# TheRealShamsaba/KnightVision

Hardware: AMD Instinct MI355X
Metric: MCTS simulations/sec + self-play games/hour (higher is better)
Workload: dtype fp32

## Files before the change

### include/kv.h

```cpp
#ifndef KV_H
#define KV_H

#include <stddef.h>
#include <stdint.h>

#ifdef __cplusplus
extern "C" {
#endif

#define KV_OK 0
#define KV_EINVAL -1
#define KV_ENOMEM -2
#define KV_EHIP -3
#define KV_EOVERFLOW -4

const char* kv_last_error(void);
int kv_version(void);

typedef struct kv_net kv_net;

size_t kv_net_packed_size(void);
int kv_net_create(int device, kv_net** out);
int kv_net_load(kv_net* net, const float* packed, size_t n_floats);
int kv_net_forward(kv_net* net, const float* planes_dev, int B, float* policy_dev, float* value_dev, void* stream);
// ... 174 lines not shown
size_t kv_sizeof_search_result(void);

int kv_search_advance(kv_engine* e, int n, const int32_t* edge , int8_t* states_out );
int kv_search_continue(kv_engine* e, int n, const kv_search_params* p, kv_search_result* out ,
                       int32_t* kept );
int kv_search_tree_size(kv_engine* e, int i, int32_t* nodes, int32_t* edges);


int kv_dev_valid_moves(int device, const int8_t* states, int n, uint16_t* moves_out, int cap, int* n_moves,
                       int8_t* states_after, uint8_t* in_check);
int kv_dev_attacks(int device, const int8_t* states, int n, uint64_t* attacked);
int kv_dev_make_move(int device, int8_t* states, const int* index, int n);
int kv_dev_dirichlet(int device, const uint64_t* seeds, int n, double alpha, int k, int draws, double* out,
                     int64_t* attempts, double* tail);
int kv_dev_eval_cache(int device, int entries, const int8_t* boards, const uint16_t* moves, const int* counts,
                      const uint32_t* logits, const uint32_t* values, int n_rows, const int* step_len, int n_steps,
                      int32_t* hit, uint32_t* out_logits, uint32_t* out_values, int64_t* counters);
int kv_host_libm(int op, const double* x, const double* y, int n, double* out);
int kv_dev_py_random(int device, const uint64_t* seeds, int n, int count, double* out);
int kv_dev_wino88i(int device, const double* V, int rows, const double* U, int K, int digits, int seg, double* M,
                   int8_t* v_digits, int* v_exp);
int kv_dev_wino88i32_out(int device, const float* M, int rows, const float* scale, const float* shift,
                         const float* resid, int fused, float* Y, int8_t* v_digits, int* v_exp);
int kv_dev_tower_front(int device, const int8_t* boards, int nb, int rows, const float* wT, const float* scale,
                       const float* shift, int fused, int8_t* v_digits, int* v_exp);
int kv_dev_tower_back(int device, const float* M, int rows, const float* scale, const float* shift,
                      const float* resid, const float* heads, int fused, float* pfeat, float* value);
int kv_dev_wino88r_out(int device, const double* M, int rows, const float* scale, const float* shift,
                       const float* resid, int fused, float* Y, int8_t* v_digits, int* v_exp);
int kv_dev_net_pair(kv_net* a, kv_net* b, int cu_share, int follow);
int kv_dev_i8gemm_bench(int device, int rows, int K, int variant, int iters, float* avg_us, float* M_out);
int kv_dev_gemm_clock(int device, int rows, int digits, double seconds, double* out);
int kv_dev_out_phases(int device, int rows, int resid, int r3, unsigned long long* stamps, float* us);

#define KV_PGN_OUTCOME_NONE (-128)
typedef struct kv_pgn_record {
    char fen[100];
    char san[12];
    int32_t outcome;
    int32_t game;
} kv_pgn_record;
int kv_pgn_extract(const char* text, size_t len, kv_pgn_record* out, size_t cap, size_t* n_out, size_t* consumed,
                   int64_t* n_games);
int kv_fen_codes(const char* fens, size_t stride, int n, int8_t* codes);
int kv_san_move_index(const char* fens, size_t fen_stride, const char* sans, size_t san_stride, int n,
                      int32_t* out);
int kv_chess_perft(const char* fen, int depth, uint64_t* nodes);
int kv_chess_san(const char* fen, const char* san_in, char* san_out, size_t san_cap, char* fen_after, size_t fen_cap);
int kv_chess_fen(const char* fen_in, char* fen_out, size_t cap);

int kv_tr_conv3x3_f16(const void* x_dev, int n, int ci, const void* w_dev, const float* bias_dev, int co,
                      void* y_dev, void* stream);
int kv_tr_conv3x3_add_f16(const void* x_dev, int n, int ci, const void* w_dev, const float* bias_dev, int co,
                          const void* add_dev, void* y_dev, void* stream);
int kv_tr_conv_weights_f16(const float* w_dev, int co, int ci_real, int ci, void* wf_dev, void* wt_dev, void* stream);
size_t kv_tr_wgrad_workspace(int n, int ci, int co, int* splits);
int kv_tr_conv3x3_wgrad_f16(const void* dy_dev, const void* x_dev, int n, int ci, int ci_real, int co, float* dw_dev,
                            void* ws_dev, size_t ws_bytes, void* stream);
size_t kv_tr_bn_workspace(int rows, int C);
int kv_tr_bn_stats_f16(const void* x_dev, int rows, int C, float eps, float* mean_dev, float* var_dev,
                       float* invstd_dev, void* ws_dev, size_t ws_bytes, void* stream);
int kv_tr_bn_apply_f16(const void* x_dev, int rows, int C, const float* mean_dev, const float* invstd_dev,
                       const float* gamma_dev, const float* beta_dev, const void* res_dev, int relu, void* y_dev,
                       void* stream);
int kv_tr_bn_backward_f16(const void* x_dev, const void* dy_dev, const void* y_dev, int rows, int C, int relu,
                          const float* mean_dev, const float* invstd_dev, const float* gamma_dev, float* dgamma_dev,
// ... 23 lines not shown
```

### knightvision_amd/_lib.py

```python
from __future__ import annotations

import ctypes as C
import os

HERE = os.path.dirname(os.path.abspath(__file__))
LIB_PATH = os.environ.get("KV_LIB_PATH") or os.path.join(HERE, "libkv.so")

_lib = None


class KVError(RuntimeError):
    pass


class Config(C.Structure):
    _fields_ = [("device", C.c_int), ("slots", C.c_int), ("n_games", C.c_int64), ("game_id_base", C.c_int64),
                ("game_id_stride", C.c_int64), ("seed", C.c_uint64), ("seed_mode", C.c_int),
                ("max_moves", C.c_int), ("batch", C.c_int), ("eps", C.c_double), ("alpha", C.c_double),
                ("sims", C.c_int), ("c_puct", C.c_float), ("eval_mode", C.c_int), ("record_cap", C.c_int64),
                ("recycle", C.c_int), ("precision", C.c_int), ("algo", C.c_int), ("tree_edge_cap", C.c_int),
                ("keep_root_visits", C.c_int), ("eval_cache", C.c_int), ("leaves", C.c_int), ("arena", C.c_int), ("sample_plies", C.c_int),
                ("sim_groups", C.c_int), ("reuse_tree", C.c_int)]


# ... 96 lines not shown
        "kv_run": ([vp, i64, i64], i),
        "kv_set_max_moves": ([vp, i], i),
        "kv_records": ([vp, P(Record), sz, P(sz)], i),
        "kv_games": ([vp, P(Game), sz, P(sz)], i),
        "kv_stats_get": ([vp, P(Stats)], i),
        "kv_sizeof_config": ([], sz),
        "kv_sizeof_stats": ([], sz),
        "kv_root_visits": ([vp, P(C.c_int32), sz, P(sz)], i),
        "kv_root_visits_device": ([vp, vp, sz, P(sz), vp], i),
        "kv_root_moves": ([vp, P(C.c_uint16), sz, P(sz)], i),
        "kv_root_moves_device": ([vp, vp, sz, P(sz), vp], i),
        "kv_records_device": ([vp, vp, sz, P(sz), vp], i),
        "kv_sync": ([vp], i),
        "kv_reset_records": ([vp], i),
        "kv_destroy": ([vp], None),
        "kv_search": ([vp, P(C.c_int8), i, P(SearchParams), P(SearchResult)], i),
        "kv_sizeof_search_result": ([], sz),
        "kv_search_advance": ([vp, i, P(C.c_int32), P(C.c_int8)], i),
        "kv_search_continue": ([vp, i, P(SearchParams), P(SearchResult), P(C.c_int32)], i),
        "kv_search_tree_size": ([vp, i, P(C.c_int32), P(C.c_int32)], i),
        "kv_dev_valid_moves": ([i, P(C.c_int8), i, P(C.c_uint16), i, P(i), P(C.c_int8), P(C.c_uint8)], i),
        "kv_dev_make_move": ([i, P(C.c_int8), P(i), i], i),
        "kv_dev_attacks": ([i, P(C.c_int8), i, P(C.c_uint64)], i),
        "kv_dev_dirichlet": ([i, P(C.c_uint64), i, C.c_double, i, i, P(C.c_double), P(i64), P(C.c_double)], i),
        "kv_dev_py_random": ([i, P(C.c_uint64), i, i, P(C.c_double)], i),
        "kv_dev_eval_cache": ([i, i, P(C.c_int8), P(C.c_uint16), P(i), P(C.c_uint32), P(C.c_uint32), i, P(i), i,
                               P(C.c_int32), P(C.c_uint32), P(C.c_uint32), P(i64)], i),
        "kv_host_libm": ([i, P(C.c_double), P(C.c_double), i, P(C.c_double)], i),
        "kv_dev_wino88i": ([i, P(C.c_double), i, P(C.c_double), i, i, i, P(C.c_double), P(C.c_int8), P(i)], i),
        "kv_dev_i8gemm_bench": ([i, i, i, i, i, P(C.c_float), P(C.c_float)], i),
        "kv_dev_gemm_clock": ([i, i, i, C.c_double, P(C.c_double)], i),
        "kv_dev_net_pair": ([vp, vp, i, i], i),
        "kv_dev_out_phases": ([i, i, i, i, P(C.c_uint64), P(C.c_float)], i),
        "kv_dev_wino88i32_out": ([i, P(C.c_float), i, P(C.c_float), P(C.c_float), P(C.c_float), i, P(C.c_float),
                                  P(C.c_int8), P(i)], i),
        "kv_dev_tower_front": ([i, P(C.c_int8), i, i, P(C.c_float), P(C.c_float), P(C.c_float), i, P(C.c_int8),
                                P(i)], i),
        "kv_dev_tower_back": ([i, P(C.c_float), i, P(C.c_float), P(C.c_float), P(C.c_float), P(C.c_float), i,
                               P(C.c_float), P(C.c_float)], i),
        "kv_dev_wino88r_out": ([i, P(C.c_double), i, P(C.c_float), P(C.c_float), P(C.c_float), i, P(C.c_float),
                                P(C.c_int8), P(i)], i),
        "kv_pgn_extract": ([C.c_char_p, sz, P(PgnRecord), sz, P(sz), P(sz), P(i64)], i),
        "kv_fen_codes": ([C.c_char_p, sz, i, P(C.c_int8)], i),
        "kv_san_move_index": ([C.c_char_p, sz, C.c_char_p, sz, i, P(C.c_int32)], i),
        "kv_chess_perft": ([C.c_char_p, i, P(C.c_uint64)], i),
        "kv_chess_san": ([C.c_char_p, C.c_char_p, C.c_char_p, sz, C.c_char_p, sz], i),
        "kv_chess_fen": ([C.c_char_p, C.c_char_p, sz], i),
        "kv_tr_conv3x3_f16": ([vp, i, i, vp, vp, i, vp, vp], i),
        "kv_tr_conv3x3_add_f16": ([vp, i, i, vp, vp, i, vp, vp, vp], i),
        "kv_tr_conv_weights_f16": ([vp, i, i, i, vp, vp, vp], i),
        "kv_tr_wgrad_workspace": ([i, i, i, P(i)], sz),
        "kv_tr_conv3x3_wgrad_f16": ([vp, vp, i, i, i, i, vp, vp, sz, vp], i),
        "kv_tr_bn_workspace": ([i, i], sz),
        "kv_tr_bn_stats_f16": ([vp, i, i, C.c_float, vp, vp, vp, vp, sz, vp], i),
        "kv_tr_bn_apply_f16": ([vp, i, i, vp, vp, vp, vp, vp, i, vp, vp], i),
        "kv_tr_bn_backward_f16": ([vp, vp, vp, i, i, i, vp, vp, vp, vp, vp, vp, vp, vp, vp, sz, vp], i),
        "kv_tr_channel_sum_f16": ([vp, i, i, vp, vp, sz, vp], i),
        "kv_tr_planes_to_nhwc": ([vp, i, i, vp, vp], i),
        "kv_tr_head1x1_f16": ([vp, i, vp, vp, vp, vp], i),
        "kv_tr_head1x1_workspace": ([i], sz),
        "kv_tr_head1x1_backward_f16": ([vp, vp, i, vp, vp, vp, vp, vp, sz, vp], i),
        "kv_tr_policy_loss_f16": ([vp, vp, vp, vp, vp, i, vp, vp, vp, vp], i),
        "kv_tr_policy_loss_backward_f16": ([vp, vp, vp, vp, vp, i, vp, vp, vp, vp, vp, vp], i),
    }
    for name, (args, res) in sig.items():
        if not hasattr(L, name):
            continue
        f = getattr(L, name)
        f.argtypes = args
        f.restype = res
    return L


EXPORTED = ["kv_last_error", "kv_version", "kv_net_packed_size", "kv_net_create", "kv_net_load", "kv_net_forward",
            "kv_net_forward_boards", "kv_net_forward_boards_legal", "kv_net_set_timing", "kv_net_last_timing", "kv_net_destroy", "kv_net_set_precision", "kv_net_set_algo",
            "kv_net_calibration", "kv_engine_calibration",
            "kv_create", "kv_sim_groups_for",
            "kv_load_weights", "kv_load_weights_b", "kv_engine_calibration_b", "kv_run", "kv_set_max_moves", "kv_records", "kv_games", "kv_stats_get", "kv_sizeof_config", "kv_sizeof_stats", "kv_root_visits", "kv_root_visits_device", "kv_root_moves", "kv_root_moves_device", "kv_records_device", "kv_sync", "kv_reset_records", "kv_destroy",
            "kv_search", "kv_sizeof_search_result", "kv_search_advance", "kv_search_continue", "kv_search_tree_size",
            "kv_dev_valid_moves", "kv_dev_make_move", "kv_dev_attacks", "kv_dev_dirichlet", "kv_dev_py_random", "kv_host_libm", "kv_dev_eval_cache",
            "kv_dev_wino88i", "kv_dev_wino88i32_out", "kv_dev_wino88r_out", "kv_dev_tower_front", "kv_dev_tower_back", "kv_dev_i8gemm_bench",
            "kv_dev_gemm_clock", "kv_dev_out_phases", "kv_dev_net_pair",
            "kv_pgn_extract", "kv_fen_codes", "kv_san_move_index", "kv_chess_perft", "kv_chess_san", "kv_chess_fen",
            "kv_tr_conv3x3_f16", "kv_tr_conv3x3_add_f16", "kv_tr_conv_weights_f16", "kv_tr_wgrad_workspace", "kv_tr_conv3x3_wgrad_f16",
            "kv_tr_bn_workspace", "kv_tr_bn_stats_f16", "kv_tr_bn_apply_f16", "kv_tr_bn_backward_f16",
            "kv_tr_channel_sum_f16", "kv_tr_planes_to_nhwc", "kv_tr_head1x1_f16", "kv_tr_head1x1_workspace",
            "kv_tr_head1x1_backward_f16", "kv_tr_policy_loss_f16", "kv_tr_policy_loss_backward_f16"]


def lib():
    global _lib
    if _lib is None:
        import torch
        if not os.path.exists(LIB_PATH):
            raise KVError(f"{LIB_PATH} is missing: run `python -c 'import __graft_entry__ as g; g.build()'` "
                          "(the HIP library is required; there is no CPU fallback)")
        L = _declare(C.CDLL(LIB_PATH))
        if hasattr(L, "kv_sizeof_search_result"):
            assert L.kv_sizeof_search_result() == C.sizeof(SearchResult), "kv_search_result: ctypes mirror differs"
        if hasattr(L, "kv_sizeof_config"):
            assert L.kv_sizeof_config() == C.sizeof(Config), "kv_config: ctypes mirror differs"
            assert L.kv_sizeof_stats() == C.sizeof(Stats), "kv_stats: ctypes mirror differs"
        _lib = L
    return _lib


def check(rc: int, what: str = ""):
    if rc != 0:
        msg = lib().kv_last_error().decode(errors="replace")
        raise KVError(f"{what} failed ({rc}): {msg}")
```

### knightvision_amd/csrc/kv_nn.hip

```cpp
#include <hip/hip_runtime.h>
#include <math.h>
#include <stdarg.h>
#include <stdlib.h>
#include <string.h>

#include <algorithm>
#include <chrono>
#include <mutex>
#include <set>
#include <utility>
#include <vector>

#include "kv_common.h"
#include "kv_wino.h"
#include "kv_wino88.h"
#include "kv_wino88d.h"
#include "kv_wino88i.h"
#include "kv_ref64.h"

namespace kv {

static thread_local char g_err[512];

void set_error(const char* fmt, ...) {
// ... 2547 lines not shown
    kv::DevEvent e0, e1;
    KV_HIP(e0.create());
    KV_HIP(e1.create());
    for (int it = 0; it < 4; ++it) {
        if (it == 3) KV_HIP(hipEventRecord(e0.e, 0));
        if (resid && r3)
            hipLaunchKernelGGL((kv::wino88i32_out_kernel<true, true, 512, true, true>), dim3(1, rows), dim3(1024), 0, 0,
                               dm.p, rows, dsc.p, dsh.p, dy.p, dy.p, v8.p, ev.p, 0, 0);
        else if (resid)
            hipLaunchKernelGGL((kv::wino88i32_out_kernel<true, true, 512, false, true>), dim3(1, rows), dim3(1024), 0,
                               0, dm.p, rows, dsc.p, dsh.p, dy.p, dy.p, v8.p, ev.p, 0, 0);
        else if (r3)
            hipLaunchKernelGGL((kv::wino88i32_out_kernel<false, false, 512, true, true>), dim3(1, rows), dim3(1024), 0,
                               0, dm.p, rows, dsc.p, dsh.p, nullptr, nullptr, v8.p, ev.p, 0, 0);
        else
            hipLaunchKernelGGL((kv::wino88i32_out_kernel<false, false, 512, false, true>), dim3(1, rows), dim3(1024), 0,
                               0, dm.p, rows, dsc.p, dsh.p, nullptr, nullptr, v8.p, ev.p, 0, 0);
        KV_HIP(hipGetLastError());
    }
    KV_HIP(hipEventRecord(e1.e, 0));
    KV_HIP(hipEventSynchronize(e1.e));
    float ms = 0.f;
    KV_HIP(hipEventElapsedTime(&ms, e0.e, e1.e));
    *us = 1000.f * ms;
    const int nb = rows < kv::kOutStampBoards ? rows : kv::kOutStampBoards;
    std::vector<unsigned long long> h((size_t)kv::kOutStampBoards * 16);
    KV_HIP(hipMemcpyFromSymbol(h.data(), HIP_SYMBOL(kv::kOutStamps), h.size() * sizeof(unsigned long long)));
    for (int b = 0; b < nb; ++b)
        for (int w = 0; w < 2; ++w)
            for (int k = 0; k < 6; ++k) stamps[((size_t)b * 2 + w) * 6 + k] = h[((size_t)b * 2 + w) * 8 + k];
    return KV_OK;
}

int kv_dev_net_pair(kv_net* a, kv_net* b, int cu_share, int follow) {
    KV_REQUIRE(a && b && a != b && cu_share >= 1 && cu_share <= 2, KV_EINVAL, "kv_dev_net_pair: bad argument");
    KV_REQUIRE(a->device == b->device, KV_EINVAL, "kv_dev_net_pair: the nets are on different devices");
    KV_HIP(hipSetDevice(a->device));
    a->cu_share = b->cu_share = cu_share;
    a->leader = nullptr;
    b->leader = follow ? a : nullptr;
    if (follow)
        for (int l = 1; l < 12; ++l)
            if (!a->gemm_done[l]) KV_HIP(hipEventCreateWithFlags(&a->gemm_done[l], hipEventDisableTiming));
    return KV_OK;
}

int kv_net_set_timing(kv_net* net, int enable) {
    KV_REQUIRE(net, KV_EINVAL, "kv_net_set_timing: NULL");
    net->timing = enable != 0;
    return KV_OK;
}

int kv_net_last_timing(kv_net* net, float* conv_ms, int* n_conv) {
    KV_REQUIRE(net && net->timing, KV_EINVAL, "kv_net_last_timing: timing not enabled");
    KV_HIP(hipEventSynchronize(net->ev[2]));
    float ms = 0.f;
    KV_HIP(hipEventElapsedTime(&ms, net->ev[1], net->ev[2]));
    if (conv_ms) *conv_ms = ms;
    if (n_conv) *n_conv = 10;
    return KV_OK;
}

void kv_net_destroy(kv_net* net) {
    if (!net || net->view) return;
    (void)hipSetDevice(net->device);
    (void)hipFree(net->w);
// ... 105 lines not shown
```

### knightvision_amd/csrc/kv_wino88.h

```cpp
#pragma once
#include <hip/hip_runtime.h>

#include "kv_common.h"
#include "kv_wino.h"

namespace kv {

constexpr int W88_XI = 100;

__device__ inline void w88_bt(const float* d, float* o) {
#pragma clang fp contract(off)
    o[0] = __builtin_fmaf(1.0f, d[8], __builtin_fmaf(-6.362500190734863f, d[6], __builtin_fmaf(10.802399635314941f, d[4], __builtin_fmaf(-5.5696001052856445f, d[2], 0.6399999856948853f * d[0]))));
    o[1] = __builtin_fmaf(1.0f, d[8], __builtin_fmaf(0.4000000059604645f, d[7], __builtin_fmaf(-6.202499866485596f, d[6], __builtin_fmaf(-2.4809999465942383f, d[5], __builtin_fmaf(9.8100004196167f, d[4], __builtin_fmaf(3.9240000247955322f, d[3], __builtin_fmaf(-4.0f, d[2], -1.600000023841858f * d[1])))))));
    o[2] = __builtin_fmaf(1.0f, d[8], __builtin_fmaf(-0.4000000059604645f, d[7], __builtin_fmaf(-6.202499866485596f, d[6], __builtin_fmaf(2.4809999465942383f, d[5], __builtin_fmaf(9.8100004196167f, d[4], __builtin_fmaf(-3.9240000247955322f, d[3], __builtin_fmaf(-4.0f, d[2], 1.600000023841858f * d[1])))))));
    o[3] = __builtin_fmaf(1.0f, d[8], __builtin_fmaf(0.800000011920929f, d[7], __builtin_fmaf(-5.722499847412109f, d[6], __builtin_fmaf(-4.578000068664551f, d[5], __builtin_fmaf(7.139999866485596f, d[4], __builtin_fmaf(5.711999893188477f, d[3], __builtin_fmaf(-1.0f, d[2], -0.800000011920929f * d[1])))))));
    o[4] = __builtin_fmaf(1.0f, d[8], __builtin_fmaf(-0.800000011920929f, d[7], __builtin_fmaf(-5.722499847412109f, d[6], __builtin_fmaf(4.578000068664551f, d[5], __builtin_fmaf(7.139999866485596f, d[4], __builtin_fmaf(-5.711999893188477f, d[3], __builtin_fmaf(-1.0f, d[2], 0.800000011920929f * d[1])))))));
    o[5] = __builtin_fmaf(1.0f, d[8], __builtin_fmaf(1.25f, d[7], __builtin_fmaf(-4.800000190734863f, d[6], __builtin_fmaf(-6.0f, d[5], __builtin_fmaf(3.3024001121520996f, d[4], __builtin_fmaf(4.127999782562256f, d[3], __builtin_fmaf(-0.40959998965263367f, d[2], -0.5120000243186951f * d[1])))))));
    o[6] = __builtin_fmaf(1.0f, d[8], __builtin_fmaf(-1.25f, d[7], __builtin_fmaf(-4.800000190734863f, d[6], __builtin_fmaf(6.0f, d[5], __builtin_fmaf(3.3024001121520996f, d[4], __builtin_fmaf(-4.127999782562256f, d[3], __builtin_fmaf(-0.40959998965263367f, d[2], 0.5120000243186951f * d[1])))))));
    o[7] = __builtin_fmaf(1.0f, d[8], __builtin_fmaf(2.0f, d[7], __builtin_fmaf(-2.362499952316284f, d[6], __builtin_fmaf(-4.724999904632568f, d[5], __builtin_fmaf(1.3523999452590942f, d[4], __builtin_fmaf(2.7047998905181885f, d[3], __builtin_fmaf(-0.1599999964237213f, d[2], -0.3199999928474426f * d[1])))))));
    o[8] = __builtin_fmaf(1.0f, d[8], __builtin_fmaf(-2.0f, d[7], __builtin_fmaf(-2.362499952316284f, d[6], __builtin_fmaf(4.724999904632568f, d[5], __builtin_fmaf(1.3523999452590942f, d[4], __builtin_fmaf(-2.7047998905181885f, d[3], __builtin_fmaf(-0.1599999964237213f, d[2], 0.3199999928474426f * d[1])))))));
    o[9] = __builtin_fmaf(1.0f, d[9], __builtin_fmaf(-6.362500190734863f, d[7], __builtin_fmaf(10.802399635314941f, d[5], __builtin_fmaf(-5.5696001052856445f, d[3], 0.6399999856948853f * d[1]))));
}

__device__ inline void w88_at(const float* d, float* o) {
// ... 154 lines not shown
#pragma clang fp contract(off)
    constexpr int C = 512;
    const size_t xs = (size_t)rows * C;
    const size_t base = (size_t)b * C + c;
    float tmp[8][10];
#pragma unroll
    for (int j = 0; j < 10; ++j) {
        float col[10], o[8];
#pragma unroll
        for (int i = 0; i < 10; ++i) col[i] = __builtin_nontemporal_load(&M[(size_t)(i * 10 + j) * xs + base]);
        w88_at(col, o);
#pragma unroll
        for (int i = 0; i < 8; ++i) tmp[i][j] = o[i];
    }
    float res[64];
#pragma unroll
    for (int p = 0; p < 64; ++p) res[p] = RESID ? resid[((size_t)b * 64 + p) * C + c] : 0.f;
#pragma unroll
    for (int i = 0; i < 8; ++i) {
        float o[8];
        w88_at(tmp[i], o);
#pragma unroll
        for (int j = 0; j < 8; ++j) {
            const int p = i * 8 + j;
            float v = o[j] * sc + sh;
            if (RESID) v += res[p];
            v = v > 0.f ? v : 0.f;
            if (WRITE_Y) Y[((size_t)b * 64 + p) * C + c] = v;
            x[p] = v;
        }
    }
}

#ifndef KV_OUT_M_NT
#define KV_OUT_M_NT 1
#endif
template <bool RESID, bool WRITE_Y, bool STAGED = false, int ABL = 0, bool YNT = false>
__device__ inline void wino88_out_plane_half(const float* __restrict__ M, int rows, int b, int c, int h, float sc,
                                             float sh, const float* resid, float* Y, float (&x2)[4][8]) {
#pragma clang fp contract(off)
    constexpr int C = 512;
    const unsigned xs = (unsigned)rows * C;
    const unsigned base = (unsigned)b * C + c;
    float t[8][5];
    unsigned rbase = (unsigned)b * 64 * C + c;
    if constexpr (STAGED) {
        unsigned mb = base;
#pragma unroll
        for (int jj = 0; jj < 5; ++jj) {
            const int j = 5 * h + jj;
            float col[10];
#pragma unroll
            for (int i = 0; i < 10; ++i) col[i] = __builtin_nontemporal_load(&M[(unsigned)(i * 10 + j) * xs + mb]);
            float o[8];
            w88_at(col, o);
#pragma unroll
            for (int i = 0; i < 8; ++i) t[i][jj] = o[i];
            asm volatile("" : "+v"(mb) : "v"(o[0]), "v"(o[7]));
        }
        asm volatile("" : "+v"(rbase) : "v"(t[0][4]), "v"(t[7][4]));
    } else if constexpr (ABL == 1) {
        const int wv = (int)(threadIdx.x >> 6), ln = (int)(threadIdx.x & 63);
        f32x4 q[13];
#pragma unroll
        for (int k = 0; k < 13; ++k) {
            const int g = wv * 13 + k, xi = (g >> 1) < 99 ? (g >> 1) : 99;
            q[k] = __builtin_nontemporal_load(
                (const f32x4*)&M[(unsigned)xi * xs + (unsigned)b * C + (unsigned)((g & 1) * 256 + 4 * ln)]);
        }
#pragma unroll
        for (int jj = 0; jj < 5; ++jj) {
            float col[10], o[8];
#pragma unroll
            for (int i = 0; i < 10; ++i) col[i] = q[(jj * 10 + i) >> 2][(jj * 10 + i) & 3];
            w88_at(col, o);
#pragma unroll
            for (int i = 0; i < 8; ++i) t[i][jj] = o[i];
        }
    } else {
#pragma unroll
        for (int jj = 0; jj < 5; ++jj) {
            const int j = 5 * h + jj;
            float col[10], o[8];
#pragma unroll
            for (int i = 0; i < 10; ++i)
                col[i] = KV_OUT_M_NT ? __builtin_nontemporal_load(&M[(unsigned)(i * 10 + j) * xs + base])
                                     : M[(unsigned)(i * 10 + j) * xs + base];
            w88_at(col, o);
#pragma unroll
            for (int i = 0; i < 8; ++i) t[i][jj] = o[i];
        }
    }
#pragma unroll
    for (int ii = 0; ii < 4; ++ii) {
        float row[10];
#pragma unroll
        for (int jj = 0; jj < 5; ++jj) {
            float lo = t[ii][jj], hi = t[4 + ii][jj];
            half_swap(lo, hi);
            row[jj] = lo;
            row[5 + jj] = hi;
        }
        float o[8];
        w88_at(row, o);
        const int i = 4 * h + ii;
        float res[8];
#pragma unroll
        for (int j = 0; j < 8; ++j)
            res[j] = RESID ? (YNT ? __builtin_nontemporal_load(&resid[(unsigned)(i * 8 + j) * C + rbase])
                                          : resid[(unsigned)(i * 8 + j) * C + rbase])
                           : 0.f;
#pragma unroll
        for (int j = 0; j < 8; ++j) {
            float v = o[j] * sc + sh;
            if (RESID) v += res[j];
            v = v > 0.f ? v : 0.f;
            if (WRITE_Y) {
                if (YNT)
                    __builtin_nontemporal_store(v, &Y[((unsigned)b * 64 + i * 8 + j) * C + c]);
                else
                    Y[((unsigned)b * 64 + i * 8 + j) * C + c] = v;
            }
            x2[ii][j] = v;
        }
        if (STAGED) asm volatile("" : "+v"(rbase) : "v"(x2[ii][0]), "v"(x2[ii][7]));
    }
}

template <bool RESID, bool WRITE_Y, bool NEXT_V>
__global__ __launch_bounds__(256) void wino88_out_kernel(const float* __restrict__ M, int rows,
                                                         const float* __restrict__ scale,
                                                         const float* __restrict__ shift, const float* resid, float* Y,
                                                         float* __restrict__ Vn) {
    constexpr int C = 512;
    const int c = blockIdx.x * 256 + threadIdx.x, b = blockIdx.y;
    float x[64];
    wino88_out_plane<RESID, WRITE_Y>(M, rows, b, c, scale[c], shift[c], resid, Y, x);
    if (NEXT_V) wino88_input_plane(x, Vn, (size_t)b * C + c, (size_t)rows * C);
}

}
```

### knightvision_amd/csrc/kv_wino88i.h

```cpp
#pragma once
#include <hip/hip_runtime.h>

#include "kv_common.h"
#include "kv_wino88.h"
#include "kv_wino88d.h"

namespace kv {

constexpr int kI8Digits = 5;
constexpr int kI8DigitsF32 = 4;

typedef int i8x16_t __attribute__((ext_vector_type(4)));
typedef int i32x16_t __attribute__((ext_vector_type(16)));

__device__ inline int i8_row_exponent(unsigned m) {
    if (!m) return 0;
    return (int)(m >> 20) - 1022 + ((m & 0xFE000u) == 0xFE000u ? 1 : 0);
}

__device__ inline int i8_row_exponent_f32(unsigned m) {
    if (!m) return 0;
    return (int)(m >> 23) - 126 + ((m & 0x7F0000u) == 0x7F0000u ? 1 : 0);
}

// ... 1610 lines not shown
        const int xi = threadIdx.x, a = xi / 10, bb = xi % 10, hh = a / 5, aa = a % 5;
        unsigned m = 0;
#pragma unroll
        for (int ww = 0; ww < NW; ++ww) m = red[ww][hh][aa][bb] > m ? red[ww][hh][aa][bb] : m;
        const int e = i8f32_row_exponent<R3>(m);
        exs[xi] = e;
        ex[(size_t)xi * rows + b] = e;
    }
    __syncthreads();
    const int q = lane & 3;
    const unsigned off0 = ((unsigned)(c >> 5) * rows + b) * kI8LineBytes<R3> + q * 32 + (c & 28),
                   xstride = NK * rows * kI8LineBytes<R3>;
    unsigned* const dst = (unsigned*)V8;
#pragma unroll
    for (int aa = 0; aa < 5; ++aa) {
        float o[10];
        wino88_input_row_of_cols(xc, aa, o);
        const int a = 5 * h + aa;
#pragma unroll
        for (int bb = 0; bb < 10; ++bb) {
            const int xi = a * 10 + bb;
            const unsigned P = i8f32_digits<R3>(o[bb], exs[xi]);
            {
                const unsigned T4 = i8_quad_transpose(P, lane);
                if constexpr (!R3)
                    __builtin_nontemporal_store(T4, &dst[(off0 + (unsigned)xi * xstride) >> 2]);
                else if (q < 3)
                    dst[(off0 + (unsigned)xi * xstride) >> 2] = T4;
            }
        }
    }
}

constexpr int kOutStampBoards = 4096;
__device__ unsigned long long kOutStamps[kOutStampBoards][2][8];

template <bool RESID, bool WRITE_Y, int CW, bool R3 = false, bool STAMP = false, int ABL = 0, bool YNT = false>
__global__ __launch_bounds__(2 * CW) void wino88i32_out_kernel(const float* __restrict__ M, int rows,
                                                               const float* __restrict__ scale,
                                                               const float* __restrict__ shift, const float* resid,
                                                               float* Y, int8_t* __restrict__ V8,
                                                               int* __restrict__ ex, int stag, int first) {
#pragma clang fp contract(off)
    static_assert(CW == 512 || CW == 256, "a row or a 256-channel segment per workgroup");
    constexpr int NK = 512 / 32, NW = CW / 32, NSEG = 512 / CW;
    __shared__ __attribute__((aligned(16))) unsigned red[NW][2][5][16];
    __shared__ int exs[100];
    const int lane = threadIdx.x & 63, w = threadIdx.x >> 6, h = lane >> 5;
    const int seg = blockIdx.x, c = seg * CW + w * 32 + (lane & 31), b = out_board<R3>((int)blockIdx.y);
    out_stagger(b, stag, first);
    unsigned long long st[6] = {};
    const bool stamper = STAMP && (w == 0 || w == NW - 1) && lane == 0 && b < kOutStampBoards;
    if constexpr (STAMP) st[0] = __builtin_amdgcn_s_memtime();
    float vk[5][10];
    {
        float t2[10][4];
        {
            float x2[4][8];
            wino88_out_plane_half<RESID, WRITE_Y, false, ABL, YNT>(M, rows, b, c, h, scale[c], shift[c], resid, Y, x2);
            wino88_input_cols(x2, h, t2);
        }
#pragma unroll
        for (int aa = 0; aa < 5; ++aa) wino88_input_row(t2, h, aa, vk[aa]);
    }
    if constexpr (STAMP) {
#pragma unroll
        for (int aa = 0; aa < 5; ++aa)
#pragma unroll
            for (int bb = 0; bb < 10; ++bb) asm volatile("" ::"v"(vk[aa][bb]));
        st[1] = __builtin_amdgcn_s_memtime();
    }
#pragma unroll
    for (int aa = 0; aa < 5; ++aa) {
        const float (&o)[10] = vk[aa];
        unsigned m[10];
#pragma unroll
        for (int bb = 0; bb < 10; ++bb) m[bb] = i8_half_max_dpp(__float_as_uint(o[bb]) & 0x7fffffffu);
        if ((lane & 31) == 16) {
            uint4* rr = (uint4*)&red[w][h][aa][0];
            rr[0] = make_uint4(m[0], m[1], m[2], m[3]);
            rr[1] = make_uint4(m[4], m[5], m[6], m[7]);
            *(uint2*)&red[w][h][aa][8] = make_uint2(m[8], m[9]);
        }
    }
    __syncthreads();
    if constexpr (STAMP) st[2] = __builtin_amdgcn_s_memtime();
    if (threadIdx.x < 100) {
        const int xi = threadIdx.x, a = xi / 10, bb = xi % 10, hh = a / 5, aa = a % 5;
        unsigned m = 0;
#pragma unroll
        for (int ww = 0; ww < NW; ++ww) m = red[ww][hh][aa][bb] > m ? red[ww][hh][aa][bb] : m;
        const int e = i8f32_row_exponent<R3>(m);
        exs[xi] = e;
        ex[((size_t)xi * NSEG + seg) * rows + b] = e;
    }
    __syncthreads();
    if constexpr (STAMP) st[3] = __builtin_amdgcn_s_memtime();
    const int q = lane & 3;
    const unsigned off0 = ((unsigned)(c >> 5) * rows + b) * kI8LineBytes<R3> + q * 32 + (c & 28),
                   xstride = NK * rows * kI8LineBytes<R3>;
    unsigned* const dst = (unsigned*)V8;
#pragma unroll
    for (int aa = 0; aa < 5; ++aa) {
        const int a = 5 * h + aa;
#pragma unroll
        for (int bb = 0; bb < 10; ++bb) {
            const int xi = a * 10 + bb;
            const unsigned P = i8f32_digits<R3>(vk[aa][bb], exs[xi]);
            {
                const unsigned T4 = i8_quad_transpose(P, lane);
                if constexpr (!R3)
                    __builtin_nontemporal_store(T4, &dst[(off0 + (unsigned)xi * xstride) >> 2]);
                else if (q < 3)
                    dst[(off0 + (unsigned)xi * xstride) >> 2] = T4;
            }
        }
    }
    if constexpr (STAMP) {
        st[4] = __builtin_amdgcn_s_memtime();
        asm volatile("s_waitcnt vmcnt(0)" ::: "memory");
        st[5] = __builtin_amdgcn_s_memtime();
        if (stamper) {
            unsigned long long* o = kOutStamps[b][w == 0 ? 0 : 1];
#pragma unroll
            for (int k = 0; k < 6; ++k) o[k] = st[k];
        }
    }
}

constexpr int kStemR3Lds = 9 * 13 * 256 * 4;
__global__ __launch_bounds__(512) void stem_r3_kernel(const int8_t* __restrict__ boards, int nb, int rows,
                                                      const float* __restrict__ wT, const float* __restrict__ scale,
                                                      const float* __restrict__ shift, int8_t* __restrict__ V8,
                                                      int* __restrict__ ex) {
#pragma clang fp contract(off)
    constexpr int NK = 256 / 32, NW = 8;
    extern __shared__ __attribute__((aligned(16))) float stem_wl[];
    __shared__ int codes[100];
    __shared__ __attribute__((aligned(16))) unsigned red[NW][2][5][16];
    __shared__ int exs[100];
    const int lane = threadIdx.x & 63, w = threadIdx.x >> 6, h = lane >> 5;
    const int c = w * 32 + (lane & 31);
    for (int i = threadIdx.x; i < 9 * 13 * 256; i += 512) {
        const int r = i >> 8, code = r / 9, t = r % 9;
        stem_wl[i] = code ? wT[(size_t)(t * 12 + code - 1) * 256 + (i & 255)] : 0.f;
    }
    const float sc = scale[c], sh = shift[c];
    const int q = lane & 3;
    unsigned* const dst = (unsigned*)V8;
    const unsigned xstride = NK * (unsigned)rows * 96u;
    for (int id = blockIdx.x; id < rows; id += gridDim.x) {
        const int b = out_board<true>(id);
        __syncthreads();
        if (threadIdx.x < 100) {
            const int i = threadIdx.x, r = i / 10 - 1, f = i % 10 - 1;
            const bool in = b < nb && r >= 0 && r < 8 && f >= 0 && f < 8;
            codes[i] = in ? boards[(size_t)b * 64 + r * 8 + f] * (9 * 256) : 0;
        }
        __syncthreads();
        float vk[5][10];
        {
            float t2[10][4];
            {
                float x2[4][8];
#pragma unroll
                for (int ii = 0; ii < 4; ++ii)
#pragma unroll
                    for (int px = 0; px < 8; ++px) {
                        const int py = 4 * h + ii;
                        float acc = 0.f;
#pragma unroll
                        for (int t = 0; t < 9; ++t)
                            acc += stem_wl[codes[(py + t / 3) * 10 + px + t % 3] + t * 256 + c];
                        const float v = __builtin_fmaf(acc, sc, sh);
                        x2[ii][px] = v > 0.f ? v : 0.f;
                    }
                wino88_input_cols(x2, h, t2);
            }
#pragma unroll
            for (int aa = 0; aa < 5; ++aa) wino88_input_row(t2, h, aa, vk[aa]);
        }
#pragma unroll
        for (int aa = 0; aa < 5; ++aa) {
            unsigned m[10];
#pragma unroll
            for (int bb = 0; bb < 10; ++bb) m[bb] = i8_half_max_dpp(__float_as_uint(vk[aa][bb]) & 0x7fffffffu);
            if ((lane & 31) == 16) {
                uint4* rr = (uint4*)&red[w][h][aa][0];
                rr[0] = make_uint4(m[0], m[1], m[2], m[3]);
                rr[1] = make_uint4(m[4], m[5], m[6], m[7]);
                *(uint2*)&red[w][h][aa][8] = make_uint2(m[8], m[9]);
            }
        }
        __syncthreads();
        if (threadIdx.x < 100) {
            const int xi = threadIdx.x, a = xi / 10, bb = xi % 10, hh = a / 5, aa = a % 5;
            unsigned m = 0;
#pragma unroll
            for (int ww = 0; ww < NW; ++ww) m = red[ww][hh][aa][bb] > m ? red[ww][hh][aa][bb] : m;
            const int e = i8_row_exponent_f32r(m);
            exs[xi] = e;
            ex[(size_t)xi * rows + b] = e;
        }
        __syncthreads();
        const unsigned off0 = ((unsigned)(c >> 5) * rows + b) * 96u + q * 32 + (c & 28);
#pragma unroll
        for (int aa = 0; aa < 5; ++aa) {
            const int a = 5 * h + aa;
#pragma unroll
            for (int bb = 0; bb < 10; ++bb) {
                const int xi = a * 10 + bb;
                const unsigned P = i8_digits_r3((double)vk[aa][bb], exs[xi]);
                const unsigned T4 = i8_quad_transpose(P, lane);
                if (q < 3) dst[(off0 + (unsigned)xi * xstride) >> 2] = T4;
            }
        }
    }
}

template <bool RESID, bool WRITE_Y, bool R3 = false>
__global__ __launch_bounds__(1024) void wino88i32_outp_kernel(const float* __restrict__ M, int rows,
                                                              const float* __restrict__ scale,
                                                              const float* __restrict__ shift, const float* resid,
                                                              float* Y, int8_t* __restrict__ V8,
                                                              int* __restrict__ ex) {
#pragma clang fp contract(off)
    constexpr int NK = 512 / 32, NW = 16, NSLOT = 3, SLOT = 20 * 2048;
    extern __shared__ __attribute__((aligned(16))) char lds_outp[];
    unsigned(*red)[2][5][16] = (unsigned(*)[2][5][16])(lds_outp + NSLOT * SLOT);
    int* exs = (int*)(lds_outp + NSLOT * SLOT + NW * 2 * 5 * 16 * 4);
    const int lane = threadIdx.x & 63, w = threadIdx.x >> 6, h = lane >> 5;
    const int wu = __builtin_amdgcn_readfirstlane(w);
    const int c = w * 32 + (lane & 31);
    const int G = (int)gridDim.x;
    const int nbw = ((int)rows - (int)blockIdx.x + G - 1) / G;
    const int nsteps = 5 * nbw;
    const int npieces = wu < 8 ? 3 : 2;
    const float sc = scale[c], sh = shift[c];
    const unsigned xs = (unsigned)rows * 512;
    auto issue = [&](int t) {
        if (t >= nsteps) return;
        const int b = (int)blockIdx.x + (t / 5) * G, jj = t % 5;
        char* dst = lds_outp + (t % NSLOT) * SLOT;
#pragma unroll
        for (int k = 0; k < 3; ++k) {
            const int q = wu + 16 * k;
            if (q < 40) {
                const int r = q >> 1, hh = r / 10, i = r - 10 * hh;
                const float* src = M + (unsigned)(i * 10 + 5 * hh + jj) * xs + (unsigned)b * 512 + (q & 1) * 256 +
// ... 244 lines not shown
```

Before: 336,700.

## Rework R3 output epilogue: permlane max reduction, f32 digit cut, scalar-base addressing

The per-row max reduction before quantisation now uses permlane16_swap plus a DPP tree, so every lane ends up holding two maxima, replacing fifty separate half-wave DPP reductions. Digit quantisation is done in f32 with precomputed shifts instead of a double-precision conversion, and the quad transpose uses precomputed perm selectors. Global loads and stores use a scalar base plus a per-lane offset, aiming to cut VGPR address arithmetic. A standalone benchmark entry point with ablation variants is also added; the f32 cut could round differently from the double path.

```diff
diff --git a/include/kv.h b/include/kv.h
--- a/include/kv.h
+++ b/include/kv.h
@@ -230,6 +230,7 @@
 int kv_dev_i8gemm_bench(int device, int rows, int K, int variant, int iters, float* avg_us, float* M_out);
 int kv_dev_gemm_clock(int device, int rows, int digits, double seconds, double* out);
 int kv_dev_out_phases(int device, int rows, int resid, int r3, unsigned long long* stamps, float* us);
+int kv_dev_out_bench(int device, int rows, int resid, int abl, int iters, float* us);
 
 #define KV_PGN_OUTCOME_NONE (-128)
 typedef struct kv_pgn_record {
diff --git a/knightvision_amd/_lib.py b/knightvision_amd/_lib.py
--- a/knightvision_amd/_lib.py
+++ b/knightvision_amd/_lib.py
@@ -152,6 +152,7 @@
         "kv_dev_gemm_clock": ([i, i, i, C.c_double, P(C.c_double)], i),
         "kv_dev_net_pair": ([vp, vp, i, i], i),
         "kv_dev_out_phases": ([i, i, i, i, P(C.c_uint64), P(C.c_float)], i),
+        "kv_dev_out_bench": ([i, i, i, i, i, P(C.c_float)], i),
         "kv_dev_wino88i32_out": ([i, P(C.c_float), i, P(C.c_float), P(C.c_float), P(C.c_float), i, P(C.c_float),
                                   P(C.c_int8), P(i)], i),
         "kv_dev_tower_front": ([i, P(C.c_int8), i, i, P(C.c_float), P(C.c_float), P(C.c_float), i, P(C.c_int8),
@@ -200,7 +201,7 @@
             "kv_search", "kv_sizeof_search_result", "kv_search_advance", "kv_search_continue", "kv_search_tree_size",
             "kv_dev_valid_moves", "kv_dev_make_move", "kv_dev_attacks", "kv_dev_dirichlet", "kv_dev_py_random", "kv_host_libm", "kv_dev_eval_cache",
             "kv_dev_wino88i", "kv_dev_wino88i32_out", "kv_dev_wino88r_out", "kv_dev_tower_front", "kv_dev_tower_back", "kv_dev_i8gemm_bench",
-            "kv_dev_gemm_clock", "kv_dev_out_phases", "kv_dev_net_pair",
+            "kv_dev_gemm_clock", "kv_dev_out_phases", "kv_dev_out_bench", "kv_dev_net_pair",
             "kv_pgn_extract", "kv_fen_codes", "kv_san_move_index", "kv_chess_perft", "kv_chess_san", "kv_chess_fen",
             "kv_tr_conv3x3_f16", "kv_tr_conv3x3_add_f16", "kv_tr_conv_weights_f16", "kv_tr_wgrad_workspace", "kv_tr_conv3x3_wgrad_f16",
             "kv_tr_bn_workspace", "kv_tr_bn_stats_f16", "kv_tr_bn_apply_f16", "kv_tr_bn_backward_f16",
diff --git a/knightvision_amd/csrc/kv_nn.hip b/knightvision_amd/csrc/kv_nn.hip
--- a/knightvision_amd/csrc/kv_nn.hip
+++ b/knightvision_amd/csrc/kv_nn.hip
@@ -2603,6 +2603,61 @@
     return KV_OK;
 }
 
+}
+
+template <bool RESID, int ABL>
+static void dev_out_bench_launch(const float* M, int rows, const float* sc, const float* sh, float* y, int8_t* v8,
+                                 int* ev, int cus) {
+    hipLaunchKernelGGL((kv::wino88i32_out_kernel<RESID, RESID, 512, true, false, ABL, RESID>), dim3(1, rows),
+                       dim3(1024), 0, 0, M, rows, sc, sh, RESID ? y : nullptr, RESID ? y : nullptr, v8, ev, 0, cus);
+}
+
+extern "C" {
+
+int kv_dev_out_bench(int device, int rows, int resid, int abl, int iters, float* us) {
+    KV_REQUIRE(rows > 0 && rows % 128 == 0 && rows <= kMaxBoards && us && iters > 0 && iters <= 1000 &&
+                   (abl == 0 || abl == 4 || abl == 8),
+               KV_EINVAL, "kv_dev_out_bench: bad arguments (rows %d, abl %d, iters %d)", rows, abl, iters);
+    KV_HIP(hipSetDevice(device));
+    const size_t nm = (size_t)kv::W88_XI * rows * 512, ny = (size_t)rows * 64 * 512;
+    kv::DevBuf<float> dm, dsc, dsh, dy;
+    kv::DevBuf<int8_t> v8;
+    kv::DevBuf<int> ev;
+    KV_HIP(dm.alloc(nm));
+    KV_HIP(dsc.alloc(512));
+    KV_HIP(dsh.alloc(512));
+    KV_HIP(dy.alloc(ny));
+    KV_HIP(v8.alloc(nm * 4));
+    KV_HIP(ev.alloc((size_t)kv::W88_XI * rows));
+    hipLaunchKernelGGL(out_phase_fill_kernel, dim3((unsigned)((nm + 255) / 256)), dim3(256), 0, 0, dm.p, nm, dsc.p,
+                       dsh.p);
+    KV_HIP(hipMemset(dy.p, 0, ny * sizeof(float)));
+    KV_HIP(hipGetLastError());
+    const int cus = device_cus();
+    std::vector<kv::DevEvent> e((size_t)iters + 1);
+    for (auto& x : e) KV_HIP(x.create());
+    for (int it = -3; it < iters; ++it) {
+        if (it == 0) KV_HIP(hipEventRecord(e[0].e, 0));
+        if (resid)
+            abl == 4   ? dev_out_bench_launch<true, 4>(dm.p, rows, dsc.p, dsh.p, dy.p, v8.p, ev.p, cus)
+            : abl == 8 ? dev_out_bench_launch<true, 8>(dm.p, rows, dsc.p, dsh.p, dy.p, v8.p, ev.p, cus)
+                       : dev_out_bench_launch<true, 0>(dm.p, rows, dsc.p, dsh.p, dy.p, v8.p, ev.p, cus);
+        else
+            abl == 4   ? dev_out_bench_launch<false, 4>(dm.p, rows, dsc.p, dsh.p, dy.p, v8.p, ev.p, cus)
+            : abl == 8 ? dev_out_bench_launch<false, 8>(dm.p, rows, dsc.p, dsh.p, dy.p, v8.p, ev.p, cus)
+                       : dev_out_bench_launch<false, 0>(dm.p, rows, dsc.p, dsh.p, dy.p, v8.p, ev.p, cus);
+        KV_HIP(hipGetLastError());
+        if (it >= 0) KV_HIP(hipEventRecord(e[(size_t)it + 1].e, 0));
+    }
+    KV_HIP(hipDeviceSynchronize());
+    for (int it = 0; it < iters; ++it) {
+        float ms = 0.f;
+        KV_HIP(hipEventElapsedTime(&ms, e[(size_t)it].e, e[(size_t)it + 1].e));
+        us[it] = 1000.f * ms;
+    }
+    return KV_OK;
+}
+
 int kv_dev_net_pair(kv_net* a, kv_net* b, int cu_share, int follow) {
     KV_REQUIRE(a && b && a != b && cu_share >= 1 && cu_share <= 2, KV_EINVAL, "kv_dev_net_pair: bad argument");
     KV_REQUIRE(a->device == b->device, KV_EINVAL, "kv_dev_net_pair: the nets are on different devices");
diff --git a/knightvision_amd/csrc/kv_wino88.h b/knightvision_amd/csrc/kv_wino88.h
--- a/knightvision_amd/csrc/kv_wino88.h
+++ b/knightvision_amd/csrc/kv_wino88.h
@@ -210,6 +210,20 @@
     }
 }
 
+#ifndef KV_OUT_SADDR
+#define KV_OUT_SADDR 1
+#endif
+template <class T>
+using global_ptr = __attribute__((address_space(1))) T*;
+template <class T>
+__device__ __forceinline__ global_ptr<T> sb_ptr(T* p, size_t bytes, unsigned lane_off) {
+    size_t a = (size_t)p + bytes;
+#if KV_OUT_SADDR
+    asm("" : "+s"(a));
+#endif
+    return (global_ptr<T>)(a + lane_off);
+}
+
 #ifndef KV_OUT_M_NT
 #define KV_OUT_M_NT 1
 #endif
@@ -256,19 +270,21 @@
             for (int i = 0; i < 8; ++i) t[i][jj] = o[i];
         }
     } else {
+        const unsigned ml = (base + 5u * (unsigned)h * xs) * 4u;
 #pragma unroll
         for (int jj = 0; jj < 5; ++jj) {
-            const int j = 5 * h + jj;
             float col[10], o[8];
 #pragma unroll
-            for (int i = 0; i < 10; ++i)
-                col[i] = KV_OUT_M_NT ? __builtin_nontemporal_load(&M[(unsigned)(i * 10 + j) * xs + base])
-                                     : M[(unsigned)(i * 10 + j) * xs + base];
+            for (int i = 0; i < 10; ++i) {
+                const auto mp = sb_ptr(M, (size_t)(i * 10 + jj) * xs * 4, ml);
+                col[i] = KV_OUT_M_NT ? __builtin_nontemporal_load(mp) : *mp;
+            }
             w88_at(col, o);
 #pragma unroll
             for (int i = 0; i < 8; ++i) t[i][jj] = o[i];
         }
     }
+    const unsigned yl = (((unsigned)b * 64 + 32u * (unsigned)h) * C + (unsigned)c) * 4u;
 #pragma unroll
     for (int ii = 0; ii < 4; ++ii) {
         float row[10];
@@ -283,21 +299,37 @@
         w88_at(row, o);
         const int i = 4 * h + ii;
         float res[8];
-#pragma unroll
-        for (int j = 0; j < 8; ++j)
-            res[j] = RESID ? (YNT ? __builtin_nontemporal_load(&resid[(unsigned)(i * 8 + j) * C + rbase])
-                                          : resid[(unsigned)(i * 8 + j) * C + rbase])
-                           : 0.f;
+        if constexpr (STAGED) {
+#pragma unroll
+            for (int j = 0; j < 8; ++j)
+                res[j] = RESID ? (YNT ? __builtin_nontemporal_load(&resid[(unsigned)(i * 8 + j) * C + rbase])
+                                              : resid[(unsigned)(i * 8 + j) * C + rbase])
+                               : 0.f;
+        } else {
+#pragma unroll
+            for (int j = 0; j < 8; ++j) {
+                const auto rp = sb_ptr(resid, (size_t)(ii * 8 + j) * C * 4, yl);
+                res[j] = RESID ? (YNT ? __builtin_nontemporal_load(rp) : *rp) : 0.f;
+            }
+        }
 #pragma unroll
         for (int j = 0; j < 8; ++j) {
             float v = o[j] * sc + sh;
             if (RESID) v += res[j];
             v = v > 0.f ? v : 0.f;
             if (WRITE_Y) {
-                if (YNT)
-                    __builtin_nontemporal_store(v, &Y[((unsigned)b * 64 + i * 8 + j) * C + c]);
-                else
-                    Y[((unsigned)b * 64 + i * 8 + j) * C + c] = v;
+                if constexpr (STAGED) {
+                    if (YNT)
+                        __builtin_nontemporal_store(v, &Y[((unsigned)b * 64 + i * 8 + j) * C + c]);
+                    else
+                        Y[((unsigned)b * 64 + i * 8 + j) * C + c] = v;
+                } else {
+                    const auto yp = sb_ptr(Y, (size_t)(ii * 8 + j) * C * 4, yl);
+                    if (YNT)
+                        __builtin_nontemporal_store(v, yp);
+                    else
+                        *yp = v;
+                }
             }
             x2[ii][j] = v;
         }
diff --git a/knightvision_amd/csrc/kv_wino88i.h b/knightvision_amd/csrc/kv_wino88i.h
--- a/knightvision_amd/csrc/kv_wino88i.h
+++ b/knightvision_amd/csrc/kv_wino88i.h
@@ -1666,6 +1666,135 @@
     }
 }
 
+template <int CTRL, int N>
+__device__ __forceinline__ void r3_max_step(const unsigned (&in)[N], unsigned (&out)[(N + 1) / 2], bool up) {
+#pragma unroll
+    for (int i = 0; i < N / 2; ++i) {
+        const unsigned keep = up ? in[2 * i + 1] : in[2 * i], send = up ? in[2 * i] : in[2 * i + 1];
+        const unsigned t = (unsigned)__builtin_amdgcn_update_dpp(0, (int)send, CTRL, 0xF, 0xF, true);
+        out[i] = keep > t ? keep : t;
+    }
+    if constexpr (N % 2 != 0) {
+        const unsigned t = (unsigned)__builtin_amdgcn_update_dpp(0, (int)in[N - 1], CTRL, 0xF, 0xF, true);
+        out[N / 2] = in[N - 1] > t ? in[N - 1] : t;
+    }
+}
+
+#ifndef KV_R3_MAX_RS
+#define KV_R3_MAX_RS 1
+#endif
+#ifndef KV_R3_CUT_F32
+#define KV_R3_CUT_F32 1
+#endif
+__device__ __forceinline__ void r3_half_maxima(const float (&vk)[5][10], int lane, unsigned (&m)[2]) {
+    unsigned s25[25], s13[13], s7[7], s4[4];
+#pragma unroll
+    for (int i = 0; i < 25; ++i) {
+        const int p0 = 2 * i, p1 = 2 * i + 1;
+        const auto r = __builtin_amdgcn_permlane16_swap(__float_as_uint(vk[p0 / 10][p0 % 10]),
+                                                        __float_as_uint(vk[p1 / 10][p1 % 10]), false, false);
+        const unsigned x = r[0] & 0x7fffffffu, y = r[1] & 0x7fffffffu;
+        s25[i] = x > y ? x : y;
+    }
+    r3_max_step<0x140>(s25, s13, (lane & 8) != 0);
+    r3_max_step<0x141>(s13, s7, (lane & 4) != 0);
+    r3_max_step<0x4E>(s7, s4, (lane & 2) != 0);
+    r3_max_step<0xB1>(s4, m, (lane & 1) != 0);
+}
+
+__device__ inline int r3_max_index(int lane, int s) {
+    const int i4 = 2 * s + (lane & 1);
+    const int i7 = i4 < 3 ? 2 * i4 + ((lane >> 1) & 1) : 6;
+    const int i13 = i7 < 6 ? 2 * i7 + ((lane >> 2) & 1) : 12;
+    const int i25 = i13 < 12 ? 2 * i13 + ((lane >> 3) & 1) : 24;
+    return 2 * i25 + ((lane >> 4) & 1);
+}
+
+__device__ __forceinline__ void r3_write_maxima(const float (&vk)[5][10], int lane, unsigned* rr) {
+#if KV_R3_MAX_RS
+    unsigned m[2];
+    r3_half_maxima(vk, lane, m);
+    rr[r3_max_index(lane, 0)] = m[0];
+    rr[r3_max_index(lane, 1)] = m[1];
+#else
+    unsigned m[50];
+#pragma unroll
+    for (int i = 0; i < 50; ++i) m[i] = i8_half_max_dpp(__float_as_uint(vk[i / 10][i % 10]) & 0x7fffffffu);
+    if ((lane & 31) == 16) {
+#pragma unroll
+        for (int i = 0; i < 50; ++i) rr[i] = m[i];
+    }
+#endif
+}
+
+__device__ __forceinline__ unsigned i8_r3_cut_f32(float v, int s) {
+    const int n = (int)__builtin_rintf(__builtin_ldexpf(v, s));
+    return ((unsigned)n + 0x808080u) ^ 0x808080u;
+}
+
+__device__ __forceinline__ unsigned r3_quad_transpose(unsigned P, unsigned sel1, unsigned sel2) {
+    const unsigned q1 = (unsigned)__builtin_amdgcn_mov_dpp((int)P, 0xB1, 0xF, 0xF, false);
+    const unsigned R = __builtin_amdgcn_perm(q1, P, sel1);
+    const unsigned r2 = (unsigned)__builtin_amdgcn_mov_dpp((int)R, 0x4E, 0xF, 0xF, false);
+    return __builtin_amdgcn_perm(r2, R, sel2);
+}
+__device__ inline void r3_transpose_sel(int lane, unsigned& sel1, unsigned& sel2) {
+    sel1 = (lane & 1) ? 0x03070105u : 0x04000602u;
+    sel2 = (lane & 2) ? 0x03020706u : 0x05040100u;
+}
+
+constexpr int kR3ShiftRow = 12;
+
+template <int NW>
+__device__ __forceinline__ void r3_row_exponents(const unsigned* red, int* shifts, int* __restrict__ ex, size_t exs,
+                                                 int b) {
+    if (threadIdx.x < 100) {
+        const int xi = threadIdx.x, hh = xi / 50, v = xi % 50;
+        unsigned m = 0;
+#pragma unroll
+        for (int ww = 0; ww < NW; ++ww) m = red[ww * 100 + xi] > m ? red[ww * 100 + xi] : m;
+        const int e = i8_row_exponent_f32r(m);
+        shifts[(hh * 5 + v / 10) * kR3ShiftRow + v % 10] = 23 - e;
+        ex[(size_t)xi * exs + b] = e;
+    }
+}
+
+template <bool RAW = false>
+__device__ __forceinline__ void r3_store_digits(const float (&vk)[5][10], const int* shifts, int h, int lane,
+                                                int8_t* __restrict__ V8, unsigned vl, unsigned xstride) {
+    unsigned sel1, sel2;
+    r3_transpose_sel(lane, sel1, sel2);
+    const bool writer = (lane & 3) < 3;
+#pragma unroll
+    for (int aa = 0; aa < 5; ++aa) {
+        unsigned T[10];
+        if constexpr (RAW) {
+#pragma unroll
+            for (int bb = 0; bb < 10; ++bb) T[bb] = __float_as_uint(vk[aa][bb]);
+        } else {
+            const int* sp = shifts + (h * 5 + aa) * kR3ShiftRow;
+            const int4 s0 = *(const int4*)sp, s1 = *(const int4*)(sp + 4);
+            const int2 s2 = *(const int2*)(sp + 8);
+            const int s[10] = {s0.x, s0.y, s0.z, s0.w, s1.x, s1.y, s1.z, s1.w, s2.x, s2.y};
+#pragma unroll
+            for (int bb = 0; bb < 10; ++bb) {
+#if KV_R3_CUT_F32
+                T[bb] = r3_quad_transpose(i8_r3_cut_f32(vk[aa][bb], s[bb]), sel1, sel2);
+#else
+                T[bb] = i8_quad_transpose(i8_digits_r3((double)vk[aa][bb], 23 - s[bb]), lane);
+#endif
+            }
+        }
+        if (writer) {
+            unsigned o = vl;
+            asm("" : "+v"(o));
+#pragma unroll
+            for (int bb = 0; bb < 10; ++bb)
+                *sb_ptr((unsigned*)V8, (size_t)(aa * 10 + bb) * xstride, o) = T[bb];
+        }
+    }
+}
+
 constexpr int kOutStampBoards = 4096;
 __device__ unsigned long long kOutStamps[kOutStampBoards][2][8];
 
@@ -1677,9 +1806,11 @@
                                                                int* __restrict__ ex, int stag, int first) {
 #pragma clang fp contract(off)
     static_assert(CW == 512 || CW == 256, "a row or a 256-channel segment per workgroup");
+    static_assert((ABL & 12) == 0 || (R3 && CW == 512), "ablations 4 and 8 are of the R3 form");
     constexpr int NK = 512 / 32, NW = CW / 32, NSEG = 512 / CW;
+    constexpr bool BACK3 = R3 && CW == 512;
     __shared__ __attribute__((aligned(16))) unsigned red[NW][2][5][16];
-    __shared__ int exs[100];
+    __shared__ __attribute__((aligned(16))) int exs[BACK3 ? 2 * 5 * kR3ShiftRow : 100];
     const int lane = threadIdx.x & 63, w = threadIdx.x >> 6, h = lane >> 5;
     const int seg = blockIdx.x, c = seg * CW + w * 32 + (lane & 31), b = out_board<R3>((int)blockIdx.y);
     out_stagger(b, stag, first);
@@ -1687,11 +1818,30 @@
     const bool stamper = STAMP && (w == 0 || w == NW - 1) && lane == 0 && b < kOutStampBoards;
     if constexpr (STAMP) st[0] = __builtin_amdgcn_s_memtime();
     float vk[5][10];
-    {
+    if constexpr ((ABL & 8) != 0) {
+        const unsigned xs = (unsigned)rows * 512u, ml = ((unsigned)b * 512u + c + 5u * (unsigned)h * xs) * 4u;
+        const unsigned yl = (((unsigned)b * 64 + 32u * (unsigned)h) * 512u + (unsigned)c) * 4u;
+#pragma unroll
+        for (int jj = 0; jj < 5; ++jj)
+#pragma unroll
+            for (int i = 0; i < 10; ++i)
+                vk[jj][i] =
+                    __builtin_nontemporal_load(sb_ptr(M, (size_t)(i * 10 + jj) * xs * 4, ml));
+#pragma unroll
+        for (int ii = 0; ii < 4; ++ii)
+#pragma unroll
+            for (int j = 0; j < 8; ++j) {
+                if constexpr (RESID)
+                    vk[ii][j] += __builtin_nontemporal_load(sb_ptr(resid, (size_t)(ii * 8 + j) * 2048, yl));
+                if constexpr (WRITE_Y)
+                    __builtin_nontemporal_store(vk[ii][j], sb_ptr(Y, (size_t)(ii * 8 + j) * 2048, yl));
+            }
+    } else {
         float t2[10][4];
         {
             float x2[4][8];
-            wino88_out_plane_half<RESID, WRITE_Y, false, ABL, YNT>(M, rows, b, c, h, scale[c], shift[c], resid, Y, x2);
+            wino88_out_plane_half<RESID, WRITE_Y, false, ABL & 3, YNT>(M, rows, b, c, h, scale[c], shift[c], resid, Y,
+                                                                       x2);
             wino88_input_cols(x2, h, t2);
         }
 #pragma unroll
@@ -1704,6 +1854,19 @@
             for (int bb = 0; bb < 10; ++bb) asm volatile("" ::"v"(vk[aa][bb]));
         st[1] = __builtin_amdgcn_s_memtime();
     }
+    if constexpr (BACK3) {
+        if constexpr ((ABL & 4) == 0) {
+            r3_write_maxima(vk, lane, &red[0][0][0][0] + (w * 2 + h) * 50);
+        }
+        __syncthreads();
+        if constexpr (STAMP) st[2] = __builtin_amdgcn_s_memtime();
+        r3_row_exponents<NW>(&red[0][0][0][0], exs, ex, (size_t)rows, b);
+        __syncthreads();
+        if constexpr (STAMP) st[3] = __builtin_amdgcn_s_memtime();
+        const unsigned xstride = NK * (unsigned)rows * 96u;
+        const unsigned vl = ((unsigned)(c >> 5) * rows + b) * 96u + (lane & 3) * 32 + (c & 28) + 50u * h * xstride;
+        r3_store_digits<(ABL & 4) != 0>(vk, exs, h, lane, V8, vl, xstride);
+    } else {
 #pragma unroll
     for (int aa = 0; aa < 5; ++aa) {
         const float (&o)[10] = vk[aa];
@@ -1750,6 +1913,7 @@
             }
         }
     }
+    }
     if constexpr (STAMP) {
         st[4] = __builtin_amdgcn_s_memtime();
         asm volatile("s_waitcnt vmcnt(0)" ::: "memory");
@@ -1771,8 +1935,8 @@
     constexpr int NK = 256 / 32, NW = 8;
     extern __shared__ __attribute__((aligned(16))) float stem_wl[];
     __shared__ int codes[100];
-    __shared__ __attribute__((aligned(16))) unsigned red[NW][2][5][16];
-    __shared__ int exs[100];
+    __shared__ __attribute__((aligned(16))) unsigned red[NW * 2 * 50];
+    __shared__ __attribute__((aligned(16))) int exs[2 * 5 * kR3ShiftRow];
     const int lane = threadIdx.x & 63, w = threadIdx.x >> 6, h = lane >> 5;
     const int c = w * 32 + (lane & 31);
     for (int i = threadIdx.x; i < 9 * 13 * 256; i += 512) {
@@ -1780,8 +1944,6 @@
         stem_wl[i] = code ? wT[(size_t)(t * 12 + code - 1) * 256 + (i & 255)] : 0.f;
     }
     const float sc = scale[c], sh = shift[c];
-    const int q = lane & 3;
-    unsigned* const dst = (unsigned*)V8;
     const unsigned xstride = NK * (unsigned)rows * 96u;
     for (int id = blockIdx.x; id < rows; id += gridDim.x) {
         const int b = out_board<true>(id);
@@ -1814,41 +1976,12 @@
 #pragma unroll
             for (int aa = 0; aa < 5; ++aa) wino88_input_row(t2, h, aa, vk[aa]);
         }
-#pragma unroll
-        for (int aa = 0; aa < 5; ++aa) {
-            unsigned m[10];
-#pragma unroll
-            for (int bb = 0; bb < 10; ++bb) m[bb] = i8_half_max_dpp(__float_as_uint(vk[aa][bb]) & 0x7fffffffu);
-            if ((lane & 31) == 16) {
-                uint4* rr = (uint4*)&red[w][h][aa][0];
-                rr[0] = make_uint4(m[0], m[1], m[2], m[3]);
-                rr[1] = make_uint4(m[4], m[5], m[6], m[7]);
-                *(uint2*)&red[w][h][aa][8] = make_uint2(m[8], m[9]);
-            }
-        }
+        r3_write_maxima(vk, lane, red + (w * 2 + h) * 50);
         __syncthreads();
-        if (threadIdx.x < 100) {
-            const int xi = threadIdx.x, a = xi / 10, bb = xi % 10, hh = a / 5, aa = a % 5;
-            unsigned m = 0;
-#pragma unroll
-            for (int ww = 0; ww < NW; ++ww) m = red[ww][hh][aa][bb] > m ? red[ww][hh][aa][bb] : m;
-            const int e = i8_row_exponent_f32r(m);
-            exs[xi] = e;
-            ex[(size_t)xi * rows + b] = e;
-        }
+        r3_row_exponents<NW>(red, exs, ex, (size_t)rows, b);
         __syncthreads();
-        const unsigned off0 = ((unsigned)(c >> 5) * rows + b) * 96u + q * 32 + (c & 28);
-#pragma unroll
-        for (int aa = 0; aa < 5; ++aa) {
-            const int a = 5 * h + aa;
-#pragma unroll
-            for (int bb = 0; bb < 10; ++bb) {
-                const int xi = a * 10 + bb;
-                const unsigned P = i8_digits_r3((double)vk[aa][bb], exs[xi]);
-                const unsigned T4 = i8_quad_transpose(P, lane);
-                if (q < 3) dst[(off0 + (unsigned)xi * xstride) >> 2] = T4;
-            }
-        }
+        const unsigned vl = ((unsigned)(c >> 5) * rows + b) * 96u + (lane & 3) * 32 + (c & 28) + 50u * h * xstride;
+        r3_store_digits(vk, exs, h, lane, V8, vl, xstride);
     }
 }
 
```

Result: no change. 339,400 (median of 2 runs) (+0.8%).
